# nens/dask-geomodeling

Measured on NVIDIA B200. Metric: fused raster chain throughput (Reclassify+Clip+Step+IsData), higher is better.
Workload: dtype int16/float32->bool

## Files before the change

dask_geomodeling_b200/_native.py:

```python
import ctypes
import os
import threading
import weakref

import numpy as np

_HERE = os.path.dirname(os.path.abspath(__file__))
LIB_PATH = os.path.join(_HERE, "libgeokernels.so")

GM_HOST, GM_DEVICE = 0, 1

_DTYPE_CODES = {
    "bool": 0, "uint8": 1, "int8": 2, "uint16": 3, "int16": 4,
    "uint32": 5, "int32": 6, "int64": 7, "float32": 8, "float64": 9,
}
_CODE_DTYPES = {v: np.dtype(k) for k, v in _DTYPE_CODES.items()}


class NativeLibraryError(RuntimeError):
    pass


def dtype_code(dtype):
    name = np.dtype(dtype).name
# ... 71 lines not shown
    _fields_ = [
        ("count", ctypes.c_int64),
        ("sum", ctypes.c_double),
        ("vmin", ctypes.c_double),
        ("vmax", ctypes.c_double),
    ]


class GmWarp(ctypes.Structure):
    _fields_ = [
        ("dst_kind", ctypes.c_int32),
        ("dst_zone", ctypes.c_int32),
        ("src_kind", ctypes.c_int32),
        ("src_zone", ctypes.c_int32),
        ("dst_geo", ctypes.c_double * 6),
        ("src_geo", ctypes.c_double * 6),
        ("src_height", ctypes.c_int64),
        ("src_width", ctypes.c_int64),
        ("win_row0", ctypes.c_int64),
        ("win_col0", ctypes.c_int64),
    ]


_vp, _i, _i64, _d = ctypes.c_void_p, ctypes.c_int, ctypes.c_int64, ctypes.c_double
_P = ctypes.POINTER
SYMBOLS = {
    "gm_abi_version": (_i, []),
    "gm_init": (_i, [_i]),
    "gm_shutdown": (_i, []),
    "gm_last_error": (ctypes.c_char_p, []),
    "gm_device_info": (_i, [_P(_i), _P(_i64), _P(_i), _P(_i)]),
    "gm_launch_count": (_i64, []),
    "gm_default_stream": (_vp, []),
    "gm_stream_sync": (_i, [_vp]),
    "gm_malloc": (_i, [_P(_vp), _i64, _vp]),
    "gm_free": (_i, [_vp, _vp]),
    "gm_host_alloc": (_i, [_P(_vp), _i64]),
    "gm_host_free": (_i, [_vp]),
    "gm_host_register": (_i, [_vp, _i64]),
    "gm_host_unregister": (_i, [_vp]),
    "gm_memcpy_h2d": (_i, [_vp, _vp, _i64, _vp]),
    "gm_memcpy_d2h": (_i, [_vp, _vp, _i64, _vp]),
    "gm_memcpy_d2d": (_i, [_vp, _vp, _i64, _vp]),
    "gm_memcpy_d2h_async": (_i, [_vp, _vp, _i64, _vp]),
    "gm_stream_create": (_i, [_P(_vp)]),
    "gm_stream_destroy": (_i, [_vp]),
    "gm_memcpy2d_h2d": (_i, [_vp, _i64, _vp, _i64, _i64, _i64, _vp]),
    "gm_fill": (_i, [_vp, ctypes.c_int32, _vp, _i64, _vp]),
    "gm_eval_program": (_i, [_P(GmProgram), _P(GmArray), _P(GmArray), _i64, _vp]),
    "gm_set_eval_mode": (_i, [_i]),
    "gm_get_eval_mode": (_i, []),
    "gm_jit_source": (_i, [_P(GmProgram), _P(ctypes.c_int32), _P(ctypes.c_int32), ctypes.c_char_p, _i64,
                           _P(_i64)]),
    "gm_jit_check": (_i, [_P(GmProgram), _P(ctypes.c_int32), _P(ctypes.c_int32), _P(_i64)]),
    "gm_jit_compile_count": (_i64, []),
    "gm_resample_nn": (_i, [_P(GmArray), _P(GmArray), _vp, _d, _d, _d, _d, _vp]),
    "gm_warp_nn": (_i, [_P(GmArray), _P(GmArray), _vp, _P(GmWarp), _P(_i64), _vp]),
    "gm_hillshade": (_i, [_P(GmArray), _P(GmArray), _vp, _i, _d, _d, _d, _d, _d, _vp]),
    "gm_moving_max": (_i, [_P(GmArray), _P(GmArray), _vp, _i, _i, _vp]),
    "gm_dilate": (_i, [_P(GmArray), _P(GmArray), _vp, _i, _vp]),
    "gm_set_smooth_mode": (_i, [_i]),
    "gm_get_smooth_mode": (_i, []),
    "gm_smooth": (_i, [_P(GmArray), _P(GmArray), _vp, _i, _d, _vp, _i, _vp, _i, _i, _i, _i,
                       _d, _d, _d, _d, _vp]),
    "gm_temporal_aggregate": (_i, [_P(GmArray), _P(GmArray), _vp, _i, _i, _d, _vp, _vp, _i, _vp]),
    "gm_temporal_cumulative": (_i, [_P(GmArray), _P(GmArray), _vp, _i, _i, _vp, _vp, _vp, _i, _vp]),
    "gm_rasterize_polygons": (_i, [_P(GmPolygons), _P(_d), _vp, _vp, _P(GmArray), _vp]),
    "gm_zonal_stats": (_i, [_P(GmArray), _vp, _i, _P(GmPolygons), _P(_d), _i, _d, _vp,
                            _i64, _i64, _vp, _vp, _vp, _vp]),
    "gm_polygons_upload": (_i, [_P(GmPolygons), _P(_vp)]),
    "gm_polygons_free": (_i, [_vp]),
    "gm_zonal_values": (_i, [_P(GmArray), _vp, _i, _P(GmPolygons), _P(_d), _vp, _vp, _vp, _vp]),
    "gm_segment_order_stat": (_i, [_vp, ctypes.c_int32, _vp, _i64, _i, _d, _vp, _vp]),
    "gm_zonal_partials_device": (_i, [_P(GmArray), _vp, _i, _P(GmPolygons), _P(_d), _vp, _i64, _i64,
                                      _vp, _vp, _i, _vp]),
    "gm_zonal_finalize_device": (_i, [_vp, _vp, _i64, _i, _vp, _vp, _P(GmPolygons), _vp]),
}

_lib = None
_lib_lock = threading.Lock()
_initialised = False


def load_library():
    global _lib
    if _lib is not None:
        return _lib
    with _lib_lock:
        if _lib is not None:
            return _lib
        if not os.path.exists(LIB_PATH):
            raise NativeLibraryError(
                "{} not found: build it with `python -m dask_geomodeling_b200.csrc.build` "
                "(there is no CPU fallback)".format(LIB_PATH)
            )
        lib = ctypes.CDLL(LIB_PATH)
        for name, (restype, argtypes) in SYMBOLS.items():
            fn = getattr(lib, name)
            fn.restype = restype
            fn.argtypes = argtypes
        if lib.gm_abi_version() != 1:
            raise NativeLibraryError("libgeokernels.so ABI version mismatch")
        _lib = lib
    return _lib


# ... 263 lines not shown
```

dask_geomodeling_b200/csrc/gm_jit.cu:

```cuda
#include "gm_common.cuh"
#include "gm_jit.h"
#include <dlfcn.h>
#include <deque>
#include <memory>
#include <mutex>
#include <unordered_map>
#include <sys/stat.h>
#include <unistd.h>

namespace gm {

static const char* kPrelude =
#include "build/gm_jit_prelude.inc"
    ;

typedef struct _nvrtcProgram* nvrtcProgram;
struct Nvrtc {
  void* handle = nullptr;
  int (*CreateProgram)(nvrtcProgram*, const char*, const char*, int, const char* const*, const char* const*);
  int (*CompileProgram)(nvrtcProgram, int, const char* const*);
  int (*GetCUBINSize)(nvrtcProgram, size_t*);
  int (*GetCUBIN)(nvrtcProgram, char*);
  int (*GetProgramLogSize)(nvrtcProgram, size_t*);
  int (*GetProgramLog)(nvrtcProgram, char*);
// ... 10 lines not shown
  const char* candidates[] = {env, "libnvrtc.so.12", "/usr/local/cuda/lib64/libnvrtc.so.12",
                              "libnvrtc.so"};
  void* h = nullptr;
  for (const char* c : candidates) {
    if (!c || !*c) continue;
    h = dlopen(c, RTLD_NOW | RTLD_LOCAL);
    if (h) break;
  }
  if (!h) return fail("NVRTC (libnvrtc.so.12) not found: set GM_NVRTC_PATH or GM_EVAL=interp");
#define GM_SYM(name)                                                                   \
  *(void**)(&g_nvrtc.name) = dlsym(h, "nvrtc" #name);                                  \
  if (!g_nvrtc.name) return fail("libnvrtc lacks nvrtc" #name)
  GM_SYM(CreateProgram); GM_SYM(CompileProgram); GM_SYM(GetCUBINSize); GM_SYM(GetCUBIN);
  GM_SYM(GetProgramLogSize); GM_SYM(GetProgramLog); GM_SYM(DestroyProgram); GM_SYM(GetErrorString);
#undef GM_SYM
  g_nvrtc.handle = h;
  return 0;
}

static const char* class_type(int cls) {
  switch (cls) {
    case GM_C_I32: return "int32_t";
    case GM_C_F32: return "float";
    case GM_C_I64: return "int64_t";
    default: return "double";
  }
}
static bool class_is_float(int cls) { return cls == GM_C_F32 || cls == GM_C_F64; }
static bool class_fits(int cls, int word) { return word == 8 || cls == GM_C_I32 || cls == GM_C_F32; }

static const char* storage_type(int dt) {
  switch (dt) {
    case GM_BOOL: case GM_U8: return "uint8_t";
    case GM_I8: return "int8_t";
    case GM_U16: return "uint16_t";
    case GM_I16: return "int16_t";
    case GM_I64: case GM_F64: return "uint64_t";
    default: return "uint32_t";
  }
}

static std::string hex(uint64_t v) {
  char buf[32];
  snprintf(buf, sizeof(buf), "0x%llxULL", (unsigned long long)v);
  return buf;
}
static std::string num(long long v) { return std::to_string(v); }
static const char* tf(bool b) { return b ? "true" : "false"; }

struct JitLayout {
  int V, U;
  bool baked[GM_MAX_TABLES];
  bool in_smem[GM_MAX_TABLES];
};

static const int kBakeLimit = 2048;

static JitLayout plan_layout(const GmProgram* prog, const int* in_dtype, const int* out_dtype) {
  JitLayout L;
  int widest = 1;
  for (int i = 0; i < prog->n_inputs; ++i) widest = std::max(widest, dtype_size(in_dtype[i]));
  for (int i = 0; i < prog->n_outputs; ++i) widest = std::max(widest, dtype_size(out_dtype[i]));
  L.V = 16 / widest;
  L.U = std::max(2, 16 / L.V);
  int total = 0;
  for (int t = 0; t < prog->n_tables; ++t) total += prog->tables[t].n;
  for (int t = 0; t < GM_MAX_TABLES; ++t) {
    L.baked[t] = t < prog->n_tables && total <= kBakeLimit;
    L.in_smem[t] = L.baked[t];
  }
  return L;
}

static thread_local const GmProgram* t_bake = nullptr;
static std::string kref(int pc, int i) {
  if (t_bake) return hex(t_bake->instr[pc].k[i]);
  return "p.k[" + num(pc) + "][" + num(i) + "]";
}

static std::string operand_b(const GmInstr& in, int pc) {
  if (in.src_kind == GM_SRC_REG) return "(uint64_t)r" + num(in.src);
  if (in.src_kind == GM_SRC_INPUT) return "(uint64_t)i" + num(in.src);
  if (in.src_kind == GM_SRC_IMM) return kref(pc, 0);
  return "0ULL";
}

static std::string convert_expr(const std::string& x, int from, int to, bool nanify, const std::string& k, int word) {
  if (from == to || !class_fits(from, word) || !class_fits(to, word)) return x;
  return std::string("cvt<") + class_type(from) + ", " + class_type(to) + ", " + tf(nanify) + ">(" + x +
         ", " + k + ")";
}

static std::string table_args(const GmProgram* prog, int t) {
  const GmTable& g = prog->tables[t];
  std::string s;
  s += g.keys ? "t" + num(t) + "k" : std::string("(const int64_t*)0");
  s += ", ";
  s += g.vals ? "t" + num(t) + "v" : std::string("(const uint64_t*)0");
  s += ", ";
  s += g.hit ? "t" + num(t) + "h" : std::string("(const uint8_t*)0");
  return s;
}

static std::string emit_instruction(const GmProgram* prog, const GmInstr& in) {
  const int word = prog->word;
  const int pc = (int)(&in - prog->instr);
  const bool fa = in.flags & GM_F_ND_A, fb = in.flags & GM_F_ND_B;
  const std::string b = operand_b(in, pc);
  std::string s;
  switch (in.op) {
    case GM_OP_LOAD:
    case GM_OP_MATB: {
      std::string src = in.src_kind == GM_SRC_REG     ? "r" + num(in.src)
                        : in.src_kind == GM_SRC_INPUT ? "i" + num(in.src)
                                                      : "(S)" + kref(pc, 0);
      const bool nanify = (in.flags & GM_F_NAN) && fb;
      const std::string v = convert_expr(src, in.cls_b, in.cls_out, nanify, kref(pc, 2), word);
      s = (in.op == GM_OP_LOAD ? std::string("acc") : "r" + num(in.aux)) + " = " + v + ";";
      break;
    }
    case GM_OP_ST: s = "r" + num(in.aux) + " = acc;"; break;
    case GM_OP_OUT: s = "o" + num(in.aux) + " = acc;"; break;
    case GM_OP_CVT:
      s = "acc = " + convert_expr("acc", in.cls_a, in.cls_out, (in.flags & GM_F_NAN) && fa, kref(pc, 1), word) + ";";
      break;
    case GM_OP_ISDATA:
    case GM_OP_ISNODATA:
      if (class_fits(in.cls_a, word))
        s = std::string("acc = is_data<") + class_type(in.cls_a) + ", " + tf(fa) + ", " +
            tf(in.op == GM_OP_ISNODATA) + ">(acc, " + kref(pc, 1) + ");";
      break;
    case GM_OP_CLIP: {
      int mode = (in.flags & GM_F_B_BOOL) ? 1 : (fb ? 2 : 0);
      if (mode == 2 && !class_fits(in.cls_b, word)) mode = 0;
      s = std::string("acc = clip<") + class_type(mode == 2 ? in.cls_b : GM_C_I32) + ", " + num(mode) +
          ">(acc, " + b + ", " + kref(pc, 1) + ", " + kref(pc, 2) + ");";
      break;
    }
    case GM_OP_AND: case GM_OP_OR: case GM_OP_XOR: case GM_OP_NOT: {
      std::string y = b;
      if (in.op == GM_OP_NOT) y = "0ULL";
      else if (in.src_kind == GM_SRC_IMM) y = "(uint64_t)(" + kref(pc, 0) + " != 0)";
      s = "acc = logic<" + num(in.op) + ">(acc, " + y + ");";
      break;
    }
    case GM_OP_RECLASS: {
      const GmTable& g = prog->tables[in.aux];
      const char* A = in.cls_a == GM_C_I32 ? "int32_t" : "int64_t";
      if (in.cls_a != GM_C_I32 && word != 8) break;
      s = std::string("acc = reclass<") + A + ", " + tf(g.kind == GM_TABLE_DENSE) + ", " +
          tf(in.flags & GM_F_ND_T) + ", " + tf(in.flags & GM_F_SELECT) + ", " + tf(fa) + ", " +
          tf(in.cls_out == GM_C_F64) + ">(acc, " + table_args(prog, in.aux) + ", " + num(g.n) + ", " +
          num(g.base) + "LL, " + kref(pc, 1) + ", " + kref(pc, 3) + ");";
      break;
    }
    case GM_OP_OVERLAY:
      if (class_fits(in.cls, word) && class_fits(in.cls_out, word))
        s = std::string("acc = overlay<") + class_type(in.cls) + ", " + class_type(in.cls_out) + ", " +
            tf(in.flags & GM_F_ND_T) + ", " + tf(in.flags & GM_F_CLOSE) + ", " + tf(in.flags & GM_F_ND_FINITE) +
            ", " + num((int)in.aux) + ">(acc, " + b + ", " + kref(pc, 2) + ", " + kref(pc, 4) + ");";
      break;
    case GM_OP_EXP: case GM_OP_LOG: case GM_OP_LOG10:
      if (class_fits(in.cls, word) && class_is_float(in.cls) && in.cls == in.cls_a)
        s = "acc = transcend<" + num(in.op) + ", " + class_type(in.cls) + ", " + tf(fa) + ">(acc, " +
            kref(pc, 1) + ", " + kref(pc, 3) + ");";
      break;
    case GM_OP_MASK:
      if (class_fits(in.cls, word) && class_fits(in.cls_a, word))
        s = std::string("acc = mask<") + class_type(in.cls) + ", " + class_type(in.cls_a) + ", " +
            tf(in.flags & GM_F_ND_T) + ", " + tf(in.flags & GM_F_CLOSE) + ", " + tf(in.flags & GM_F_ND_FINITE) +
            ">(acc, " + kref(pc, 0) + ", " + kref(pc, 1) + ", " + kref(pc, 3) + ", " + kref(pc, 4) + ");";
      break;
    case GM_OP_MASKBELOW:
      if (class_fits(in.cls, word) && class_fits(in.cls_a, word))
        s = std::string("acc = mask_below<") + class_type(in.cls) + ", " + class_type(in.cls_a) + ">(acc, " +
            kref(pc, 0) + ", " + kref(pc, 5) + ");";
      break;
    case GM_OP_STEP:
      if (class_fits(in.cls, word) && class_fits(in.cls_a, word))
        s = std::string("acc = step<") + class_type(in.cls) + ", " + class_type(in.cls_a) + ", " + tf(fa) +
            ">(acc, " + kref(pc, 0) + ", " + kref(pc, 1) + ", " + kref(pc, 2) + ", " + kref(pc, 3) + ", " +
            kref(pc, 4) + ");";
      break;
    case GM_OP_CLASSIFY:
      if (class_fits(in.cls, word) && class_fits(in.cls_a, word))
        s = std::string("acc = classify<") + class_type(in.cls) + ", " + class_type(in.cls_a) + ", " + tf(fa) +
            ", " + tf(in.flags & GM_F_RIGHT) + ">(acc, t" + num(in.aux) + "k, " + num(prog->tables[in.aux].n) +
            ", " + kref(pc, 1) + ", " + kref(pc, 3) + ");";
      break;
    default: {
      if (!class_fits(in.cls, word)) break;
      const bool imm = in.src_kind == GM_SRC_IMM;
      const bool is_cmp = in.op >= GM_OP_EQ && in.op <= GM_OP_LE;
      s = std::string("acc = ") + (is_cmp ? "compare<" : "math<") + num(in.op) + ", " + class_type(in.cls) +
          ", " + tf(fa) + ", " + tf(fb && !imm) + ">(acc, " + b + ", " + kref(pc, 1) + ", " + kref(pc, 2) +
          ", " + kref(pc, 3) + ");";
      break;
    }
  }
  return s;
}

static void emit_table_data(std::string& src, const GmProgram* prog, const JitLayout& L) {
  for (int t = 0; t < prog->n_tables; ++t) {
    if (!L.baked[t]) continue;
    const GmTable& g = prog->tables[t];
    const std::string id = num(t);
    if (g.keys) {
      src += "__device__ const int64_t g_t" + id + "k[" + num(std::max(g.n, 1)) + "] = {";
      for (int i = 0; i < g.n; ++i) src += "(int64_t)" + hex(((const uint64_t*)g.keys)[i]) + ",";
      src += "};\n";
    }
    if (g.vals) {
      src += "__device__ const uint64_t g_t" + id + "v[" + num(std::max(g.n, 1)) + "] = {";
      for (int i = 0; i < g.n; ++i) src += hex(((const uint64_t*)g.vals)[i]) + ",";
      src += "};\n";
    }
    if (g.hit) {
      src += "__device__ const uint8_t g_t" + id + "h[" + num(std::max(g.n, 1)) + "] = {";
      for (int i = 0; i < g.n; ++i) src += num(g.hit[i]) + ",";
      src += "};\n";
    }
  }
}

static std::string generate(const GmProgram* prog, const int* in_dtype, const int* out_dtype,
                            const JitLayout& L) {
  const int V = L.V, U = L.U;
  std::string src;
  src.reserve(1 << 16);
  src += "#define GM_WORD " + num(prog->word) + "\n";
  src += kPrelude;
  src += "\nstruct Params { const void* in[" + num(GM_MAX_INPUTS) + "]; void* out[" + num(GM_MAX_OUTPUTS) +
         "]; long long n; const int64_t* tk[" + num(GM_MAX_TABLES) + "]; const uint64_t* tv[" +
         num(GM_MAX_TABLES) + "]; const uint8_t* th[" + num(GM_MAX_TABLES) + "]; unsigned long long k[" +
         num(GM_MAX_INSTR) + "][6]; };\n";
  emit_table_data(src, prog, L);

  std::string tab_params, tab_args;
  for (int t = 0; t < prog->n_tables; ++t) {
    const GmTable& g = prog->tables[t];
    const std::string id = num(t), n = num(std::max(g.n, 1));
    if (L.in_smem[t]) {
      if (g.keys) src += "__shared__ int64_t t" + id + "k[" + n + "];\n";
      if (g.vals) src += "__shared__ uint64_t t" + id + "v[" + n + "];\n";
      if (g.hit) src += "__shared__ uint8_t t" + id + "h[" + n + "];\n";
    } else {
      tab_params += ", const int64_t* __restrict__ t" + id + "k, const uint64_t* __restrict__ t" + id +
                    "v, const uint8_t* __restrict__ t" + id + "h";
      tab_args += ", t" + id + "k, t" + id + "v, t" + id + "h";
    }
  }

  src += "GM_DEV void pixel(const Params& p";
  bool first = false;
  for (int i = 0; i < prog->n_inputs; ++i) { src += std::string(first ? "" : ", ") + "S i" + num(i); first = false; }
  for (int i = 0; i < prog->n_outputs; ++i) { src += std::string(first ? "" : ", ") + "S& o" + num(i); first = false; }
  src += tab_params + ") {\n  S acc = 0, r0 = 0, r1 = 0, r2 = 0, r3 = 0;\n";
  for (int pc = 0; pc < prog->n_instr; ++pc) {
    const std::string line = emit_instruction(prog, prog->instr[pc]);
    if (!line.empty()) src += "  " + line + "\n";
  }
  src += "  (void)r0; (void)r1; (void)r2; (void)r3;\n}\n";

  auto words = [&](int dt) { return std::max(1, V * dtype_size(dt) / 4); };
  src += "GM_DEV void group(const Params& p";
  first = false;
  for (int i = 0; i < prog->n_inputs; ++i) { src += std::string(first ? "" : ", ") + "const uint32_t* a" + num(i); first = false; }
  for (int i = 0; i < prog->n_outputs; ++i) { src += std::string(first ? "" : ", ") + "uint32_t* w" + num(i); first = false; }
  src += tab_params + ") {\n";
  for (int j = 0; j < V; ++j) {
    src += "  {";
    for (int i = 0; i < prog->n_outputs; ++i) src += " S o" + num(i) + ";";
    src += " pixel(p";
    first = false;
    for (int i = 0; i < prog->n_inputs; ++i) {
      src += std::string(first ? "" : ", ") + "element<" + storage_type(in_dtype[i]) + ", " + num(j) + ">(a" + num(i) + ")";
      first = false;
    }
    for (int i = 0; i < prog->n_outputs; ++i) { src += std::string(first ? "" : ", ") + "o" + num(i); first = false; }
    src += tab_args + ");";
    for (int i = 0; i < prog->n_outputs; ++i)
      src += " set_element<" + num(dtype_size(out_dtype[i])) + ", " + num(j) + ">(w" + num(i) + ", o" + num(i) + ");";
    src += " }\n";
  }
  src += "}\n";

  src += "extern \"C\" __global__ void __launch_bounds__(256) gm_fused(const __grid_constant__ Params p) {\n";
  src += "  const int tid = threadIdx.x;\n";
  for (int t = 0; t < prog->n_tables; ++t) {
    const GmTable& g = prog->tables[t];
    const std::string id = num(t);
    if (L.in_smem[t]) {
      src += "  for (int i = tid; i < " + num(g.n) + "; i += 256) {";
      if (g.keys) src += " t" + id + "k[i] = g_t" + id + "k[i];";
      if (g.vals) src += " t" + id + "v[i] = g_t" + id + "v[i];";
      if (g.hit) src += " t" + id + "h[i] = g_t" + id + "h[i];";
      src += " }\n";
    } else {
      src += "  const int64_t* t" + id + "k = p.tk[" + id + "]; const uint64_t* t" + id + "v = p.tv[" + id +
             "]; const uint8_t* t" + id + "h = p.th[" + id + "];\n";
    }
  }
  if (prog->n_tables) src += "  __syncthreads();\n";
  for (int i = 0; i < prog->n_inputs; ++i)
    src += "  const unsigned char* __restrict__ in" + num(i) + " = (const unsigned char*)p.in[" + num(i) + "];\n";
  for (int i = 0; i < prog->n_outputs; ++i)
    src += "  unsigned char* __restrict__ out" + num(i) + " = (unsigned char*)p.out[" + num(i) + "];\n";
  src += "  const long long groups = p.n / " + num(V) + ";\n";
  src += "  const long long chunk = 256LL * " + num(U) + ";\n";
  src += "  const long long n_chunks = groups / chunk;\n";
  src += "  for (long long c = blockIdx.x; c < n_chunks; c += gridDim.x) {\n";
  src += "    const long long g0 = c * chunk + tid;\n";
  for (int i = 0; i < prog->n_inputs; ++i)
    src += "    uint32_t a" + num(i) + "[" + num(U) + "][" + num(words(in_dtype[i])) + "];\n";
  src += "    #pragma unroll\n    for (int u = 0; u < " + num(U) + "; ++u) {\n";
  for (int i = 0; i < prog->n_inputs; ++i) {
    const int bytes = V * dtype_size(in_dtype[i]);
    src += "      load_group<" + num(bytes) + ">(a" + num(i) + "[u], in" + num(i) + " + (g0 + u * 256LL) * " + num(bytes) + ");\n";
  }
  src += "    }\n";
  src += "    #pragma unroll\n    for (int u = 0; u < " + num(U) + "; ++u) {\n";
  for (int i = 0; i < prog->n_outputs; ++i)
    src += "      uint32_t w" + num(i) + "[" + num(words(out_dtype[i])) + "];\n";
  src += "      group(p";
  first = false;
  for (int i = 0; i < prog->n_inputs; ++i) { src += std::string(first ? "" : ", ") + "a" + num(i) + "[u]"; first = false; }
  for (int i = 0; i < prog->n_outputs; ++i) { src += std::string(first ? "" : ", ") + "w" + num(i); first = false; }
  src += tab_args + ");\n";
  for (int i = 0; i < prog->n_outputs; ++i) {
    const int bytes = V * dtype_size(out_dtype[i]);
    src += "      store_group<" + num(bytes) + ">(out" + num(i) + " + (g0 + u * 256LL) * " + num(bytes) + ", w" + num(i) + ");\n";
  }
  src += "    }\n  }\n";
  src += "  for (long long g = n_chunks * chunk + (long long)blockIdx.x * 256 + tid; g < groups; g += (long long)gridDim.x * 256) {\n";
  for (int i = 0; i < prog->n_inputs; ++i) {
    const int bytes = V * dtype_size(in_dtype[i]);
    src += "    uint32_t a" + num(i) + "[" + num(words(in_dtype[i])) + "]; load_group<" + num(bytes) + ">(a" + num(i) +
           ", in" + num(i) + " + g * " + num(bytes) + ");\n";
  }
  for (int i = 0; i < prog->n_outputs; ++i)
    src += "    uint32_t w" + num(i) + "[" + num(words(out_dtype[i])) + "];\n";
  src += "    group(p";
  first = false;
  for (int i = 0; i < prog->n_inputs; ++i) { src += std::string(first ? "" : ", ") + "a" + num(i); first = false; }
// ... 198 lines not shown
  const std::string key = program_key(prog, in_dtype, out_dtype, L);
  std::string constants;
  for (int pc = 0; pc < prog->n_instr; ++pc) constants.append((const char*)prog->instr[pc].k, sizeof(prog->instr[pc].k));
  const std::string baked_key = key + '#' + constants;
  std::shared_ptr<JitKernel> k;
  {
    std::lock_guard<std::mutex> lock(g_jit_mutex);
    auto build = [&](const std::string& as, bool bake) -> std::shared_ptr<JitKernel> {
      t_bake = bake ? prog : nullptr;
      std::string source = generate(prog, in_dtype, out_dtype, L);
      t_bake = nullptr;
      std::shared_ptr<JitKernel> fresh = std::make_shared<JitKernel>();
      fresh->key = as;
      fresh->layout = L;
      g_last_source = source;
      if (compile_kernel(source, fresh.get())) return nullptr;
      if (g_kernels.size() >= kMaxKernels && !g_kernel_order.empty()) {
        g_kernels.erase(g_kernel_order.front());
        g_kernel_order.pop_front();
      }
      g_kernels[as] = fresh;
      g_kernel_order.push_back(as);
      return fresh;
    };
    auto baked = g_kernels.find(baked_key);
    if (baked != g_kernels.end()) {
      k = baked->second;
    } else {
      auto it = g_kernels.find(key);
      k = it != g_kernels.end() ? it->second : build(key, false);
      if (!k) return 1;
      std::string& last = g_last_constants[key];
      if (n >= kBakeFromPixels && last == constants && !getenv("GM_JIT_NO_BAKE")) {
        std::shared_ptr<JitKernel> special = build(baked_key, true);
        if (special) k = special;
      }
      last = constants;
    }
  }
  JitParams p;
  memset(&p, 0, sizeof(p));
  for (int i = 0; i < prog->n_inputs; ++i) p.in[i] = in[i];
  for (int i = 0; i < prog->n_outputs; ++i) p.out[i] = out[i];
  p.n = n;
  for (int pc = 0; pc < prog->n_instr; ++pc)
    for (int i = 0; i < 6; ++i) p.k[pc][i] = prog->instr[pc].k[i];
  for (int t = 0; t < prog->n_tables; ++t) {
    p.tk[t] = (const int64_t*)tkeys[t];
    p.tv[t] = (const uint64_t*)tvals[t];
    p.th[t] = (const uint8_t*)thit[t];
  }
  const int64_t per_block = 256LL * L.U * L.V;
  int64_t grid = (n + per_block - 1) / per_block;
  const int64_t cap = (int64_t)sm_count() * k->blocks_per_sm;
  if (grid > cap) grid = cap;
  if (grid < 1) grid = 1;
  void* args[] = {&p};
  cudaError_t e = cudaLaunchKernel((const void*)k->kernel, dim3((unsigned)grid), dim3(256), args, 0, s);
  if (e != cudaSuccess) return fail(std::string("specialised kernel launch: ") + cudaGetErrorString(e));
  count_launch();
  return 0;
}

int64_t jit_compile_count() { return g_compiles.load(); }

}

using namespace gm;

extern "C" int gm_jit_source(const GmProgram* prog, const int32_t* in_dtype, const int32_t* out_dtype,
                             char* buffer, int64_t capacity, int64_t* length) {
  if (!prog || !length) return fail("gm_jit_source: null argument");
  if (prog->n_instr < 1 || prog->n_instr > GM_MAX_INSTR || prog->n_inputs > GM_MAX_INPUTS ||
      prog->n_outputs > GM_MAX_OUTPUTS || prog->n_tables > GM_MAX_TABLES)
    return fail("gm_jit_source: bad program");
  const JitLayout L = plan_layout(prog, in_dtype, out_dtype);
  const std::string source = generate(prog, in_dtype, out_dtype, L);
  *length = (int64_t)source.size();
  if (buffer && capacity > 0) {
    const size_t n = std::min((size_t)capacity - 1, source.size());
    memcpy(buffer, source.data(), n);
    buffer[n] = 0;
  }
  return 0;
}

extern "C" int gm_jit_check(const GmProgram* prog, const int32_t* in_dtype, const int32_t* out_dtype,
                            int64_t* cubin_bytes) {
  if (!prog) return fail("gm_jit_check: null program");
  const JitLayout L = plan_layout(prog, in_dtype, out_dtype);
  const std::string source = generate(prog, in_dtype, out_dtype, L);
  std::vector<char> cubin;
  std::lock_guard<std::mutex> lock(g_jit_mutex);
  if (nvrtc_compile(source, cubin)) return 1;
  if (cubin_bytes) *cubin_bytes = (int64_t)cubin.size();
  return 0;
}

extern "C" int64_t gm_jit_compile_count(void) { return jit_compile_count(); }
```

dask_geomodeling_b200/csrc/gm_jit_prelude.cuh:

```cuda

typedef signed char int8_t;
typedef unsigned char uint8_t;
typedef short int16_t;
typedef unsigned short uint16_t;
typedef int int32_t;
typedef unsigned int uint32_t;
typedef long long int64_t;
typedef unsigned long long uint64_t;

#if GM_WORD == 8
typedef uint64_t S;
#else
typedef uint32_t S;
#endif

#define GM_DEV __device__ __forceinline__

template <typename A, typename B> struct Same { static constexpr bool value = false; };
template <typename A> struct Same<A, A> { static constexpr bool value = true; };
template <typename T> struct IsFloat { static constexpr bool value = false; };
template <> struct IsFloat<float> { static constexpr bool value = true; };
template <> struct IsFloat<double> { static constexpr bool value = true; };

template <typename T> struct Raw;
template <> struct Raw<int32_t> {
  static GM_DEV int32_t get(uint64_t b) { return (int32_t)(uint32_t)b; }
  static GM_DEV uint64_t put(int32_t v) { return (uint64_t)(uint32_t)v; }
};
template <> struct Raw<float> {
  static GM_DEV float get(uint64_t b) { return __uint_as_float((uint32_t)b); }
  static GM_DEV uint64_t put(float v) { return (uint64_t)__float_as_uint(v); }
};
template <> struct Raw<int64_t> {
  static GM_DEV int64_t get(uint64_t b) { return (int64_t)b; }
  static GM_DEV uint64_t put(int64_t v) { return (uint64_t)v; }
};
template <> struct Raw<double> {
  static GM_DEV double get(uint64_t b) { return __longlong_as_double((long long)b); }
  static GM_DEV uint64_t put(double v) { return (uint64_t)__double_as_longlong(v); }
};

template <typename T> GM_DEV T quiet_nan() { return T(0); }
template <> GM_DEV float quiet_nan<float>() { return __int_as_float(0x7fc00000); }
template <> GM_DEV double quiet_nan<double>() { return __longlong_as_double(0x7ff8000000000000LL); }

template <typename ST> GM_DEV S slot_of(ST v) { return (S)v; }
template <> GM_DEV S slot_of<int8_t>(int8_t v) { return (S)(uint32_t)(int32_t)v; }
template <> GM_DEV S slot_of<int16_t>(int16_t v) { return (S)(uint32_t)(int32_t)v; }
template <> GM_DEV S slot_of<int32_t>(int32_t v) { return (S)(uint32_t)v; }

template <typename ST, int J> GM_DEV S element(const uint32_t* w) {
  if constexpr (sizeof(ST) == 8) {
    return (S)((uint64_t)w[2 * J] | ((uint64_t)w[2 * J + 1] << 32));
  } else if constexpr (sizeof(ST) == 4) {
    return slot_of<ST>((ST)w[J]);
  } else if constexpr (sizeof(ST) == 2) {
    return slot_of<ST>((ST)(uint16_t)(w[J / 2] >> (16 * (J % 2))));
  } else {
    return slot_of<ST>((ST)(uint8_t)(w[J / 4] >> (8 * (J % 4))));
  }
}

template <int SZ, int J> GM_DEV void set_element(uint32_t* w, S s) {
  if constexpr (SZ == 8) {
    w[2 * J] = (uint32_t)(uint64_t)s;
    w[2 * J + 1] = (uint32_t)((uint64_t)s >> 32);
  } else if constexpr (SZ == 4) {
    w[J] = (uint32_t)s;
  } else if constexpr (SZ == 2) {
    if constexpr (J % 2 == 0) w[J / 2] = (uint32_t)s & 0xffffu;
    else w[J / 2] |= ((uint32_t)s & 0xffffu) << 16;
  } else {
    if constexpr (J % 4 == 0) w[J / 4] = (uint32_t)s & 0xffu;
    else w[J / 4] |= ((uint32_t)s & 0xffu) << (8 * (J % 4));
  }
}

template <int BYTES> GM_DEV void load_group(uint32_t* w, const void* p) {
  if constexpr (BYTES == 16) {
    const uint4 v = __ldcs(reinterpret_cast<const uint4*>(p));
    w[0] = v.x; w[1] = v.y; w[2] = v.z; w[3] = v.w;
  } else if constexpr (BYTES == 8) {
    const uint2 v = __ldcs(reinterpret_cast<const uint2*>(p));
    w[0] = v.x; w[1] = v.y;
  } else if constexpr (BYTES == 4) {
    w[0] = __ldcs(reinterpret_cast<const unsigned int*>(p));
  } else if constexpr (BYTES == 2) {
    w[0] = __ldcs(reinterpret_cast<const unsigned short*>(p));
  } else {
    w[0] = __ldcs(reinterpret_cast<const unsigned char*>(p));
  }
}
template <int BYTES> GM_DEV void store_group(void* p, const uint32_t* w) {
  if constexpr (BYTES == 16) {
    __stcs(reinterpret_cast<uint4*>(p), make_uint4(w[0], w[1], w[2], w[3]));
  } else if constexpr (BYTES == 8) {
    __stcs(reinterpret_cast<uint2*>(p), make_uint2(w[0], w[1]));
  } else if constexpr (BYTES == 4) {
    __stcs(reinterpret_cast<unsigned int*>(p), w[0]);
  } else if constexpr (BYTES == 2) {
    __stcs(reinterpret_cast<unsigned short*>(p), (unsigned short)w[0]);
  } else {
    __stcs(reinterpret_cast<unsigned char*>(p), (unsigned char)w[0]);
  }
}

GM_DEV int32_t w_add(int32_t a, int32_t b) { return (int32_t)((uint32_t)a + (uint32_t)b); }
GM_DEV int64_t w_add(int64_t a, int64_t b) { return (int64_t)((uint64_t)a + (uint64_t)b); }
GM_DEV float w_add(float a, float b) { return a + b; }
GM_DEV double w_add(double a, double b) { return a + b; }
GM_DEV int32_t w_sub(int32_t a, int32_t b) { return (int32_t)((uint32_t)a - (uint32_t)b); }
GM_DEV int64_t w_sub(int64_t a, int64_t b) { return (int64_t)((uint64_t)a - (uint64_t)b); }
GM_DEV float w_sub(float a, float b) { return a - b; }
// ... 43 lines not shown
  OP_AND, OP_OR, OP_XOR, OP_NOT, OP_ISDATA, OP_ISNODATA, OP_OVERLAY, OP_CLIP, OP_MASK,
  OP_MASKBELOW, OP_STEP, OP_CLASSIFY, OP_RECLASS, OP_MATB
};

template <typename From, typename To, bool NANIFY> GM_DEV S cvt(S x, uint64_t k) {
  const From v = Raw<From>::get(x);
  To r = (To)v;
  if constexpr (IsFloat<To>::value && NANIFY) r = (v == Raw<From>::get(k)) ? quiet_nan<To>() : r;
  return (S)Raw<To>::put(r);
}

template <int OP, typename T, bool FA, bool FB>
GM_DEV S math(S a, uint64_t b, uint64_t k1, uint64_t k2, uint64_t k3) {
  const T x = Raw<T>::get(a), y = Raw<T>::get(b);
  T r;
  if constexpr (OP == OP_ADD) r = w_add(x, y);
  else if constexpr (OP == OP_SUB) r = w_sub(x, y);
  else if constexpr (OP == OP_RSUB) r = w_sub(y, x);
  else if constexpr (OP == OP_MUL) r = w_mul(x, y);
  else if constexpr (OP == OP_DIV) r = w_div(x, y);
  else if constexpr (OP == OP_RDIV) r = w_div(y, x);
  else if constexpr (OP == OP_POW) r = w_pow(x, y);
  else r = w_pow(y, x);
  bool bad = !finite_(r);
  if constexpr (FA) bad = bad || (x == Raw<T>::get(k1));
  if constexpr (FB) bad = bad || (y == Raw<T>::get(k2));
  return (S)Raw<T>::put(bad ? Raw<T>::get(k3) : r);
}

template <int OP, typename T, bool FA, bool FB>
GM_DEV S compare(S a, uint64_t b, uint64_t k1, uint64_t k2, uint64_t k3) {
  const T x = Raw<T>::get(a), y = Raw<T>::get(b);
  bool r;
  if constexpr (OP == OP_EQ) r = x == y;
  else if constexpr (OP == OP_NE) r = x != y;
  else if constexpr (OP == OP_GT) r = x > y;
  else if constexpr (OP == OP_GE) r = x >= y;
  else if constexpr (OP == OP_LT) r = x < y;
  else r = x <= y;
  bool bad = false;
  if constexpr (FA) bad = bad || (x == Raw<T>::get(k1));
  if constexpr (FB) bad = bad || (y == Raw<T>::get(k2));
  return bad ? (S)k3 : (S)(r ? 1u : 0u);
}

template <int OP, typename T, bool FA> GM_DEV S transcend(S a, uint64_t k1, uint64_t k3) {
  const T x = Raw<T>::get(a);
  const T r = OP == OP_EXP ? t_exp(x) : OP == OP_LOG ? t_log(x) : t_log10(x);
  bool bad = !finite_(r);
  if constexpr (FA) bad = bad || (x == Raw<T>::get(k1));
  return (S)Raw<T>::put(bad ? Raw<T>::get(k3) : r);
}

template <typename A, bool FA, bool WANT_NODATA> GM_DEV S is_data(S a, uint64_t k1) {
  bool is_nd = false;
  if constexpr (FA) is_nd = Raw<A>::get(a) == Raw<A>::get(k1);
  return (S)((is_nd == WANT_NODATA) ? 1u : 0u);
}

template <int OP> GM_DEV S logic(S a, uint64_t b) {
  const bool x = (uint32_t)a != 0u, y = (uint32_t)b != 0u;
  bool r;
  if constexpr (OP == OP_AND) r = x && y;
  else if constexpr (OP == OP_OR) r = x || y;
  else if constexpr (OP == OP_XOR) r = x != y;
  else r = !x;
  return (S)(r ? 1u : 0u);
}

template <typename B, int MODE> GM_DEV S clip(S a, uint64_t b, uint64_t k1, uint64_t k2) {
  if constexpr (MODE == 1) return ((uint32_t)b == 0u) ? (S)k1 : a;
  else if constexpr (MODE == 2) return (Raw<B>::get(b) == Raw<B>::get(k2)) ? (S)k1 : a;
  else return a;
}

template <typename T, typename A, bool HAS, bool CL, bool FIN>
GM_DEV S mask(S a, uint64_t k0, uint64_t k1, uint64_t k3, uint64_t k4) {
  const T x = (T)Raw<A>::get(a);
  bool nod = false;
  if constexpr (HAS) {
    if constexpr (CL) nod = close_(x, Raw<T>::get(k1), Raw<T>::get(k4), FIN);
    else nod = x == Raw<T>::get(k1);
  }
  return nod ? (S)k3 : (S)k0;
}

template <typename T, typename A> GM_DEV S mask_below(S a, uint64_t k0, uint64_t k5) {
  return ((T)Raw<A>::get(a) < Raw<T>::get(k0)) ? (S)k5 : a;
}

template <typename T, typename A, bool FA>
GM_DEV S step(S a, uint64_t k0, uint64_t k1, uint64_t k2, uint64_t k3, uint64_t k4) {
  const A raw = Raw<A>::get(a);
  const T x = (T)raw, loc = Raw<T>::get(k0);
  S r = a;
  r = x < loc ? (S)k2 : r;
  r = x == loc ? (S)k3 : r;
  r = x > loc ? (S)k4 : r;
  if constexpr (FA) r = (raw == Raw<A>::get(k1)) ? a : r;
  return r;
}

template <typename T, typename A, bool FA, bool RIGHT>
GM_DEV S classify(S a, const int64_t* keys, int n, uint64_t k1, uint64_t k3) {
  const A raw = Raw<A>::get(a);
  const T x = (T)raw;
  int lo = 0, hi = n;
  if (x != x) lo = n;
  else
    while (lo < hi) {
      const int mid = (lo + hi) >> 1;
      const T e = Raw<T>::get((uint64_t)keys[mid]);
      const bool go = RIGHT ? (e < x) : (e <= x);
      if (go) lo = mid + 1; else hi = mid;
    }
  if constexpr (FA) return (raw == Raw<A>::get(k1)) ? (S)k3 : (S)(uint32_t)lo;
  return (S)(uint32_t)lo;
}

template <typename T, typename To, bool HAS, bool CL, bool FIN, int KIND>
GM_DEV S overlay(S a, uint64_t b, uint64_t k2, uint64_t k4) {
  const T y = Raw<T>::get(b);
  bool nod = false;
  if constexpr (HAS) {
    if constexpr (CL) nod = close_(y, Raw<T>::get(k2), Raw<T>::get(k4), FIN);
    else nod = y == Raw<T>::get(k2);
  }
  To next = (To)y;
  if constexpr (KIND == 5) {
    next = (To)(Raw<To>::get(a) + (To)1);
  } else if constexpr (KIND != 0) {
    const To old = Raw<To>::get(a);
    if (next != next) next = old;
    else if (old == old) {
      if constexpr (KIND == 1) next = next > old ? next : old;
      else if constexpr (KIND == 2) next = next < old ? next : old;
      else if constexpr (KIND == 3) next = old + next;
      else next = old * next;
    }
  }
  return nod ? a : (S)Raw<To>::put(next);
}

template <typename A, bool DENSE, bool ND_ONLY, bool SELECT, bool FA, bool OUT_F64>
GM_DEV S reclass(S a, const int64_t* keys, const uint64_t* vals, const uint8_t* hit, int n,
                 int64_t base, uint64_t k1, uint64_t k3) {
  const int64_t key = (int64_t)Raw<A>::get(a);
  int found = 0;
  uint64_t val = k3;
  if constexpr (DENSE) {
    const uint64_t idx = (uint64_t)(key - base);
    if (idx < (uint64_t)n) {
      found = hit[idx];
      if constexpr (!ND_ONLY) val = found ? vals[idx] : val;
    }
  } else {
    int lo = 0, hi = n;
    while (lo < hi) {
      const int mid = (lo + hi) >> 1;
      if (keys[mid] < key) lo = mid + 1; else hi = mid;
    }
    if (lo < n && keys[lo] == key) {
      found = hit ? hit[lo] : 1;
      if constexpr (!ND_ONLY) val = vals[lo];
    }
  }
  if constexpr (FA) found = (key == (int64_t)k1) ? 2 : found;
  if constexpr (ND_ONLY) {
    const unsigned lut = (SELECT ? 0u : 1u) | 2u;
    return (S)((lut >> found) & 1u);
  } else {
#if GM_WORD == 8
    S keep;
    if constexpr (OUT_F64) keep = (S)Raw<double>::put((double)Raw<A>::get(a));
    else keep = (S)Raw<int64_t>::put((int64_t)Raw<A>::get(a));
    return found ? (S)val : (SELECT ? (S)k3 : keep);
#else
    return a;
#endif
  }
}
```

include/geokernels.h:

```cpp
#ifndef GEOKERNELS_H
#define GEOKERNELS_H

#include <stdint.h>

#ifdef __cplusplus
extern "C" {
#endif

#define GM_ABI_VERSION 1

enum GmDType {
  GM_BOOL = 0, GM_U8 = 1, GM_I8 = 2, GM_U16 = 3, GM_I16 = 4,
  GM_U32 = 5, GM_I32 = 6, GM_I64 = 7, GM_F32 = 8, GM_F64 = 9
};

enum GmClass { GM_C_I32 = 0, GM_C_I64 = 1, GM_C_F32 = 2, GM_C_F64 = 3 };

enum GmSpace { GM_HOST = 0, GM_DEVICE = 1 };

typedef struct GmArray {
  void*   data;
  int32_t dtype;
  int32_t space;
  int64_t shape[3];
// ... 63 lines not shown
typedef struct GmTable {
  const void* keys;
  const void* vals;
  const uint8_t* hit;
  int64_t base;
  int32_t n;
  int32_t kind;
} GmTable;

typedef struct GmProgram {
  int32_t n_instr;
  int32_t n_inputs;
  int32_t n_outputs;
  int32_t word;
  int32_t n_tables;
  int32_t reserved;
  GmInstr instr[GM_MAX_INSTR];
  GmTable tables[GM_MAX_TABLES];
} GmProgram;

int  gm_abi_version(void);
int  gm_init(int device);
int  gm_shutdown(void);
const char* gm_last_error(void);
int  gm_device_info(int* sm_count, int64_t* total_mem, int* cc_major, int* cc_minor);
int64_t gm_launch_count(void);
void* gm_default_stream(void);
int  gm_stream_sync(void* stream);

int  gm_malloc(void** ptr, int64_t bytes, void* stream);
int  gm_free(void* ptr, void* stream);
int  gm_host_alloc(void** ptr, int64_t bytes);
int  gm_host_free(void* ptr);
int  gm_host_register(void* ptr, int64_t bytes);
int  gm_host_unregister(void* ptr);
int  gm_memcpy_h2d(void* dst, const void* src, int64_t bytes, void* stream);
int  gm_memcpy_d2h(void* dst, const void* src, int64_t bytes, void* stream);
int  gm_memcpy_d2h_async(void* dst, const void* src, int64_t bytes, void* stream);
int  gm_memcpy_d2d(void* dst, const void* src, int64_t bytes, void* stream);
int  gm_stream_create(void** stream);
int  gm_stream_destroy(void* stream);
int  gm_memcpy2d_h2d(void* dst, int64_t dpitch, const void* src, int64_t spitch,
                     int64_t row_bytes, int64_t rows, void* stream);
int  gm_fill(void* dst, int32_t dtype, const void* value, int64_t count, void* stream);

int  gm_eval_program(const GmProgram* prog, const GmArray* inputs,
                     GmArray* outputs, int64_t n_pixels, void* stream);

enum GmEvalMode { GM_EVAL_AUTO = 0, GM_EVAL_INTERPRET = 1, GM_EVAL_SPECIALISE = 2 };
int  gm_set_eval_mode(int mode);
int  gm_get_eval_mode(void);
int  gm_jit_source(const GmProgram* prog, const int32_t* in_dtype, const int32_t* out_dtype,
                   char* buffer, int64_t capacity, int64_t* length);
int  gm_jit_check(const GmProgram* prog, const int32_t* in_dtype, const int32_t* out_dtype,
                  int64_t* cubin_bytes);
int64_t gm_jit_compile_count(void);

int  gm_resample_nn(const GmArray* src, GmArray* dst, const void* nodata,
                    double col0, double col_step, double row0, double row_step,
                    void* stream);

enum GmCrsKind { GM_CRS_GEOGRAPHIC = 0, GM_CRS_MERCATOR = 1, GM_CRS_UTM = 2 };
typedef struct GmWarp {
  int32_t dst_kind, dst_zone;
  int32_t src_kind, src_zone;
  double  dst_geo[6];
  double  src_geo[6];
  int64_t src_height, src_width;
  int64_t win_row0, win_col0;
} GmWarp;
int  gm_warp_nn(const GmArray* src, GmArray* dst, const void* nodata, const GmWarp* warp,
                int64_t* misses, void* stream);

int  gm_hillshade(const GmArray* src, GmArray* dst, const void* nodata, int has_nodata,
                  double fill, double xres, double yres, double altitude_deg,
                  double azimuth_deg, void* stream);
int  gm_moving_max(const GmArray* src, GmArray* dst, const void* nodata, int has_nodata,
                   int size, void* stream);
int  gm_dilate(const GmArray* src, GmArray* dst, const void* values, int n_values,
               void* stream);
enum GmSmoothMode { GM_SMOOTH_EXACT = 0, GM_SMOOTH_FMA = 1, GM_SMOOTH_FLOAT32 = 2 };
int  gm_set_smooth_mode(int mode);
int  gm_get_smooth_mode(void);
int  gm_smooth(const GmArray* src, GmArray* dst, const void* nodata, int has_nodata,
               double fill, const double* wy, int ly, const double* wx, int lx,
               int my, int mx, int zoom, double zy, double zx, double oy, double ox,
               void* stream);

enum GmStat { GM_STAT_SUM = 0, GM_STAT_COUNT, GM_STAT_MIN, GM_STAT_MAX, GM_STAT_MEAN,
              GM_STAT_MEDIAN, GM_STAT_STD, GM_STAT_VAR, GM_STAT_PERCENTILE };
int  gm_temporal_aggregate(const GmArray* src, GmArray* dst, const void* nodata, int has_nodata,
                           int stat, double q, const int32_t* bin_offsets,
                           const int32_t* frame_index, int n_bins, void* stream);
int  gm_temporal_cumulative(const GmArray* src, GmArray* dst, const void* nodata, int has_nodata,
                            int stat, const int32_t* bin_offsets, const int32_t* frame_index,
                            const int32_t* out_frame, int n_bins, void* stream);

typedef struct GmPolygons {
  const double*  xy;
  const int64_t* ring_offsets;
  const int64_t* poly_offsets;
  int64_t n_polygons;
  int64_t n_rings;
  int64_t n_vertices;
  const void* resident;
} GmPolygons;
// ... 35 lines not shown
```

Before: 833.4.

## Bake small reclass tables as bitmasks, fold IsData into Step, pack bool outputs

Small dense reclassify tables that only yield boolean hits are encoded as two 32-bit immediate bitmasks, so they no longer need shared-memory staging. A Step followed by IsData/IsNoData is fused into one expression that maps the branches straight to data flags. Byte outputs are packed four at a time into one 32-bit store, and the grid is no longer capped at the resident block count when no shared tables exist. The price is more code-generation special cases, and the Step fold only fires when constants are baked.

```diff
diff --git a/dask_geomodeling_b200/_native.py b/dask_geomodeling_b200/_native.py
--- a/dask_geomodeling_b200/_native.py
+++ b/dask_geomodeling_b200/_native.py
@@ -147,6 +147,8 @@
     "gm_get_eval_mode": (_i, []),
     "gm_jit_source": (_i, [_P(GmProgram), _P(ctypes.c_int32), _P(ctypes.c_int32), ctypes.c_char_p, _i64,
                            _P(_i64)]),
+    "gm_jit_baked_source": (_i, [_P(GmProgram), _P(ctypes.c_int32), _P(ctypes.c_int32), ctypes.c_char_p, _i64,
+                                 _P(_i64)]),
     "gm_jit_check": (_i, [_P(GmProgram), _P(ctypes.c_int32), _P(ctypes.c_int32), _P(_i64)]),
     "gm_jit_compile_count": (_i64, []),
     "gm_resample_nn": (_i, [_P(GmArray), _P(GmArray), _vp, _d, _d, _d, _d, _vp]),
diff --git a/dask_geomodeling_b200/csrc/gm_jit.cu b/dask_geomodeling_b200/csrc/gm_jit.cu
--- a/dask_geomodeling_b200/csrc/gm_jit.cu
+++ b/dask_geomodeling_b200/csrc/gm_jit.cu
@@ -86,9 +86,25 @@
   int V, U;
   bool baked[GM_MAX_TABLES];
   bool in_smem[GM_MAX_TABLES];
+  bool bits[GM_MAX_TABLES];
 };
 
 static const int kBakeLimit = 2048;
+static const int kBitsLimit = 64;
+
+static bool bits_table(const GmProgram* prog, int t) {
+  const GmTable& g = prog->tables[t];
+  if (g.kind != GM_TABLE_DENSE || !g.hit || g.n < 1 || g.n > kBitsLimit || g.base < INT32_MIN ||
+      g.base + g.n - 1 > INT32_MAX)
+    return false;
+  for (int pc = 0; pc < prog->n_instr; ++pc) {
+    const GmInstr& in = prog->instr[pc];
+    if ((in.op == GM_OP_RECLASS || in.op == GM_OP_CLASSIFY) && in.aux == t &&
+        (in.op != GM_OP_RECLASS || !(in.flags & GM_F_ND_T) || in.cls_a != GM_C_I32))
+      return false;
+  }
+  return true;
+}
 
 static JitLayout plan_layout(const GmProgram* prog, const int* in_dtype, const int* out_dtype) {
   JitLayout L;
@@ -101,7 +117,8 @@
   for (int t = 0; t < prog->n_tables; ++t) total += prog->tables[t].n;
   for (int t = 0; t < GM_MAX_TABLES; ++t) {
     L.baked[t] = t < prog->n_tables && total <= kBakeLimit;
-    L.in_smem[t] = L.baked[t];
+    L.bits[t] = L.baked[t] && bits_table(prog, t);
+    L.in_smem[t] = L.baked[t] && !L.bits[t];
   }
   return L;
 }
@@ -136,12 +153,23 @@
   return s;
 }
 
-static std::string emit_instruction(const GmProgram* prog, const GmInstr& in) {
+static const GmInstr* folded_is_data(const GmProgram* prog, int pc) {
+  const GmInstr& in = prog->instr[pc];
+  if (!t_bake || pc + 1 >= prog->n_instr) return nullptr;
+  const GmInstr& nd = prog->instr[pc + 1];
+  const bool producer = in.op == GM_OP_STEP;
+  const bool is_data = nd.op == GM_OP_ISDATA || nd.op == GM_OP_ISNODATA;
+  return producer && is_data && (nd.flags & GM_F_ND_A) && class_fits(nd.cls_a, prog->word) ? &nd : nullptr;
+}
+
+static std::string emit_instruction(const GmProgram* prog, const GmInstr& in, const JitLayout& L,
+                                    const GmInstr* fold) {
   const int word = prog->word;
   const int pc = (int)(&in - prog->instr);
   const bool fa = in.flags & GM_F_ND_A, fb = in.flags & GM_F_ND_B;
   const std::string b = operand_b(in, pc);
-  std::string s;
+  const std::string arm = fold ? std::string(", IsNd<") + class_type(fold->cls_a) + ">{" + kref(pc + 1, 1) + "}" : "";
+  std::string s, call;
   switch (in.op) {
     case GM_OP_LOAD:
     case GM_OP_MATB: {
@@ -182,6 +210,14 @@
       const GmTable& g = prog->tables[in.aux];
       const char* A = in.cls_a == GM_C_I32 ? "int32_t" : "int64_t";
       if (in.cls_a != GM_C_I32 && word != 8) break;
+      if (L.bits[in.aux]) {
+        const unsigned lut = ((in.flags & GM_F_SELECT) ? 0u : 1u) | 2u;
+        uint32_t w[2] = {0, 0};
+        for (int i = 0; i < g.n; ++i) w[i / 32] |= ((lut >> g.hit[i]) & 1u) << (i % 32);
+        s = std::string("acc = reclass_bits<") + tf(in.flags & GM_F_SELECT) + ", " + tf(fa) + ">(acc, " +
+            num(w[0]) + "u, " + num(w[1]) + "u, " + num(g.n) + "u, " + num(g.base) + ", " + kref(pc, 1) + ");";
+        break;
+      }
       s = std::string("acc = reclass<") + A + ", " + tf(g.kind == GM_TABLE_DENSE) + ", " +
           tf(in.flags & GM_F_ND_T) + ", " + tf(in.flags & GM_F_SELECT) + ", " + tf(fa) + ", " +
           tf(in.cls_out == GM_C_F64) + ">(acc, " + table_args(prog, in.aux) + ", " + num(g.n) + ", " +
@@ -212,9 +248,9 @@
       break;
     case GM_OP_STEP:
       if (class_fits(in.cls, word) && class_fits(in.cls_a, word))
-        s = std::string("acc = step<") + class_type(in.cls) + ", " + class_type(in.cls_a) + ", " + tf(fa) +
-            ">(acc, " + kref(pc, 0) + ", " + kref(pc, 1) + ", " + kref(pc, 2) + ", " + kref(pc, 3) + ", " +
-            kref(pc, 4) + ");";
+        call = std::string("step<") + class_type(in.cls) + ", " + class_type(in.cls_a) + ", " + tf(fa) +
+               ">(acc, " + kref(pc, 0) + ", " + kref(pc, 1) + ", " + kref(pc, 2) + ", " + kref(pc, 3) + ", " +
+               kref(pc, 4) + arm + ")";
       break;
     case GM_OP_CLASSIFY:
       if (class_fits(in.cls, word) && class_fits(in.cls_a, word))
@@ -232,12 +268,15 @@
       break;
     }
   }
+  if (!call.empty())
+    s = fold ? std::string("acc = data_flag<") + tf(fold->op == GM_OP_ISNODATA) + ">(" + call + ");"
+             : "acc = " + call + ";";
   return s;
 }
 
 static void emit_table_data(std::string& src, const GmProgram* prog, const JitLayout& L) {
   for (int t = 0; t < prog->n_tables; ++t) {
-    if (!L.baked[t]) continue;
+    if (!L.in_smem[t]) continue;
     const GmTable& g = prog->tables[t];
     const std::string id = num(t);
     if (g.keys) {
@@ -275,6 +314,7 @@
   for (int t = 0; t < prog->n_tables; ++t) {
     const GmTable& g = prog->tables[t];
     const std::string id = num(t), n = num(std::max(g.n, 1));
+    if (L.bits[t]) continue;
     if (L.in_smem[t]) {
       if (g.keys) src += "__shared__ int64_t t" + id + "k[" + n + "];\n";
       if (g.vals) src += "__shared__ uint64_t t" + id + "v[" + n + "];\n";
@@ -292,8 +332,10 @@
   for (int i = 0; i < prog->n_outputs; ++i) { src += std::string(first ? "" : ", ") + "S& o" + num(i); first = false; }
   src += tab_params + ") {\n  S acc = 0, r0 = 0, r1 = 0, r2 = 0, r3 = 0;\n";
   for (int pc = 0; pc < prog->n_instr; ++pc) {
-    const std::string line = emit_instruction(prog, prog->instr[pc]);
+    const GmInstr* fold = folded_is_data(prog, pc);
+    const std::string line = emit_instruction(prog, prog->instr[pc], L, fold);
     if (!line.empty()) src += "  " + line + "\n";
+    if (fold && !line.empty()) ++pc;
   }
   src += "  (void)r0; (void)r1; (void)r2; (void)r3;\n}\n";
 
@@ -303,20 +345,27 @@
   for (int i = 0; i < prog->n_inputs; ++i) { src += std::string(first ? "" : ", ") + "const uint32_t* a" + num(i); first = false; }
   for (int i = 0; i < prog->n_outputs; ++i) { src += std::string(first ? "" : ", ") + "uint32_t* w" + num(i); first = false; }
   src += tab_params + ") {\n";
+  auto packed = [&](int i) { return dtype_size(out_dtype[i]) == 1 && V % 4 == 0; };
   for (int j = 0; j < V; ++j) {
-    src += "  {";
-    for (int i = 0; i < prog->n_outputs; ++i) src += " S o" + num(i) + ";";
-    src += " pixel(p";
+    src += "  ";
+    for (int i = 0; i < prog->n_outputs; ++i) src += "S o" + num(i) + "_" + num(j) + "; ";
+    src += "pixel(p";
     first = false;
     for (int i = 0; i < prog->n_inputs; ++i) {
       src += std::string(first ? "" : ", ") + "element<" + storage_type(in_dtype[i]) + ", " + num(j) + ">(a" + num(i) + ")";
       first = false;
     }
-    for (int i = 0; i < prog->n_outputs; ++i) { src += std::string(first ? "" : ", ") + "o" + num(i); first = false; }
+    for (int i = 0; i < prog->n_outputs; ++i) { src += std::string(first ? "" : ", ") + "o" + num(i) + "_" + num(j); first = false; }
     src += tab_args + ");";
-    for (int i = 0; i < prog->n_outputs; ++i)
-      src += " set_element<" + num(dtype_size(out_dtype[i])) + ", " + num(j) + ">(w" + num(i) + ", o" + num(i) + ");";
-    src += " }\n";
+    for (int i = 0; i < prog->n_outputs; ++i) {
+      const std::string o = "o" + num(i) + "_" + num(j), w = "w" + num(i);
+      if (!packed(i))
+        src += " set_element<" + num(dtype_size(out_dtype[i])) + ", " + num(j) + ">(" + w + ", " + o + ");";
+      else if (j % 4 == 3)
+        src += " " + w + "[" + num(j / 4) + "] = pack_bytes(o" + num(i) + "_" + num(j - 3) + ", o" + num(i) + "_" +
+               num(j - 2) + ", o" + num(i) + "_" + num(j - 1) + ", " + o + ");";
+    }
+    src += "\n";
   }
   src += "}\n";
 
@@ -325,6 +374,7 @@
   for (int t = 0; t < prog->n_tables; ++t) {
     const GmTable& g = prog->tables[t];
     const std::string id = num(t);
+    if (L.bits[t]) continue;
     if (L.in_smem[t]) {
       src += "  for (int i = tid; i < " + num(g.n) + "; i += 256) {";
       if (g.keys) src += " t" + id + "k[i] = g_t" + id + "k[i];";
@@ -629,7 +679,9 @@
   }
   const int64_t per_block = 256LL * L.U * L.V;
   int64_t grid = (n + per_block - 1) / per_block;
-  const int64_t cap = (int64_t)sm_count() * k->blocks_per_sm;
+  bool smem_tables = false;
+  for (int t = 0; t < prog->n_tables; ++t) smem_tables = smem_tables || L.in_smem[t];
+  const int64_t cap = smem_tables ? (int64_t)sm_count() * k->blocks_per_sm : (int64_t)INT32_MAX;
   if (grid > cap) grid = cap;
   if (grid < 1) grid = 1;
   void* args[] = {&p};
@@ -645,14 +697,16 @@
 
 using namespace gm;
 
-extern "C" int gm_jit_source(const GmProgram* prog, const int32_t* in_dtype, const int32_t* out_dtype,
-                             char* buffer, int64_t capacity, int64_t* length) {
+static int jit_source(const GmProgram* prog, const int32_t* in_dtype, const int32_t* out_dtype, bool bake,
+                      char* buffer, int64_t capacity, int64_t* length) {
   if (!prog || !length) return fail("gm_jit_source: null argument");
   if (prog->n_instr < 1 || prog->n_instr > GM_MAX_INSTR || prog->n_inputs > GM_MAX_INPUTS ||
       prog->n_outputs > GM_MAX_OUTPUTS || prog->n_tables > GM_MAX_TABLES)
     return fail("gm_jit_source: bad program");
   const JitLayout L = plan_layout(prog, in_dtype, out_dtype);
+  t_bake = bake ? prog : nullptr;
   const std::string source = generate(prog, in_dtype, out_dtype, L);
+  t_bake = nullptr;
   *length = (int64_t)source.size();
   if (buffer && capacity > 0) {
     const size_t n = std::min((size_t)capacity - 1, source.size());
@@ -660,6 +714,16 @@
     buffer[n] = 0;
   }
   return 0;
+}
+
+extern "C" int gm_jit_source(const GmProgram* prog, const int32_t* in_dtype, const int32_t* out_dtype,
+                             char* buffer, int64_t capacity, int64_t* length) {
+  return jit_source(prog, in_dtype, out_dtype, false, buffer, capacity, length);
+}
+
+extern "C" int gm_jit_baked_source(const GmProgram* prog, const int32_t* in_dtype, const int32_t* out_dtype,
+                                   char* buffer, int64_t capacity, int64_t* length) {
+  return jit_source(prog, in_dtype, out_dtype, true, buffer, capacity, length);
 }
 
 extern "C" int gm_jit_check(const GmProgram* prog, const int32_t* in_dtype, const int32_t* out_dtype,
diff --git a/dask_geomodeling_b200/csrc/gm_jit_prelude.cuh b/dask_geomodeling_b200/csrc/gm_jit_prelude.cuh
--- a/dask_geomodeling_b200/csrc/gm_jit_prelude.cuh
+++ b/dask_geomodeling_b200/csrc/gm_jit_prelude.cuh
@@ -59,6 +59,11 @@
   } else {
     return slot_of<ST>((ST)(uint8_t)(w[J / 4] >> (8 * (J % 4))));
   }
+}
+
+GM_DEV uint32_t pack_bytes(S s0, S s1, S s2, S s3) {
+  return ((uint32_t)s0 & 0xffu) | ((uint32_t)s1 & 0xffu) << 8 | ((uint32_t)s2 & 0xffu) << 16 |
+         ((uint32_t)s3 & 0xffu) << 24;
 }
 
 template <int SZ, int J> GM_DEV void set_element(uint32_t* w, S s) {
@@ -208,11 +213,21 @@
   return (S)Raw<T>::put(bad ? Raw<T>::get(k3) : r);
 }
 
+template <bool WANT_NODATA> GM_DEV S data_flag(bool is_nd) { return (S)((is_nd == WANT_NODATA) ? 1u : 0u); }
+
 template <typename A, bool FA, bool WANT_NODATA> GM_DEV S is_data(S a, uint64_t k1) {
   bool is_nd = false;
   if constexpr (FA) is_nd = Raw<A>::get(a) == Raw<A>::get(k1);
-  return (S)((is_nd == WANT_NODATA) ? 1u : 0u);
-}
+  return data_flag<WANT_NODATA>(is_nd);
+}
+
+struct Id {
+  GM_DEV S operator()(uint64_t v) const { return (S)v; }
+};
+template <typename C> struct IsNd {
+  uint64_t nd;
+  GM_DEV bool operator()(uint64_t v) const { return Raw<C>::get(v) == Raw<C>::get(nd); }
+};
 
 template <int OP> GM_DEV S logic(S a, uint64_t b) {
   const bool x = (uint32_t)a != 0u, y = (uint32_t)b != 0u;
@@ -245,15 +260,15 @@
   return ((T)Raw<A>::get(a) < Raw<T>::get(k0)) ? (S)k5 : a;
 }
 
-template <typename T, typename A, bool FA>
-GM_DEV S step(S a, uint64_t k0, uint64_t k1, uint64_t k2, uint64_t k3, uint64_t k4) {
+template <typename T, typename A, bool FA, typename F = Id>
+GM_DEV auto step(S a, uint64_t k0, uint64_t k1, uint64_t k2, uint64_t k3, uint64_t k4, F f = F()) {
   const A raw = Raw<A>::get(a);
   const T x = (T)raw, loc = Raw<T>::get(k0);
-  S r = a;
-  r = x < loc ? (S)k2 : r;
-  r = x == loc ? (S)k3 : r;
-  r = x > loc ? (S)k4 : r;
-  if constexpr (FA) r = (raw == Raw<A>::get(k1)) ? a : r;
+  auto r = f(a);
+  r = x < loc ? f(k2) : r;
+  r = x == loc ? f(k3) : r;
+  r = x > loc ? f(k4) : r;
+  if constexpr (FA) r = (raw == Raw<A>::get(k1)) ? f(a) : r;
   return r;
 }
 
@@ -336,3 +351,14 @@
 #endif
   }
 }
+
+template <bool SELECT, bool FA>
+GM_DEV S reclass_bits(S a, uint32_t lo, uint32_t hi, uint32_t n, int32_t base, uint64_t k1) {
+  const unsigned lut = (SELECT ? 0u : 1u) | 2u;
+  const int32_t key = Raw<int32_t>::get(a);
+  const uint32_t idx = (uint32_t)key - (uint32_t)base;
+  const uint32_t w = idx < 32u ? lo : hi;
+  unsigned r = idx < n ? (w >> (idx & 31u)) & 1u : lut & 1u;
+  if constexpr (FA) r = (key == (int32_t)k1 && (int64_t)k1 == (int64_t)(int32_t)k1) ? (lut >> 2) & 1u : r;
+  return (S)r;
+}
diff --git a/include/geokernels.h b/include/geokernels.h
--- a/include/geokernels.h
+++ b/include/geokernels.h
@@ -139,6 +139,8 @@
 int  gm_get_eval_mode(void);
 int  gm_jit_source(const GmProgram* prog, const int32_t* in_dtype, const int32_t* out_dtype,
                    char* buffer, int64_t capacity, int64_t* length);
+int  gm_jit_baked_source(const GmProgram* prog, const int32_t* in_dtype, const int32_t* out_dtype,
+                         char* buffer, int64_t capacity, int64_t* length);
 int  gm_jit_check(const GmProgram* prog, const int32_t* in_dtype, const int32_t* out_dtype,
                   int64_t* cubin_bytes);
 int64_t gm_jit_compile_count(void);
```

Result: faster. 891.0, median of 6 (+6.9%).
